# SIMPLE-BuildingSimulation/heat

Measured on AMD Instinct MI355X. Metric: surface-node-updates/sec, higher is better.
Workload: dtype f64

## Files before the change

### heat_amd/csrc/kernels.hip

```cpp
#include <hip/hip_runtime.h>

#include <algorithm>
#include <atomic>
#include <cstdlib>

#include "device_math.hpp"
#include "kernels.hpp"
#include "layout.hpp"

namespace heat {

__device__ __forceinline__ void eval_side(const SideConst &c, const StepWeather &w, double air_t, double rad_alt,
                                          double rad_out, double surf_t, double &hs, double &rad_t, int &bad) {
    const double natural = tarp_natural(air_t, surf_t, c.cos_eff, bad);
    if ((c.kind_n & 3) == KIND_OUTDOOR) {
        const bool windward = (c.kind_n & 4) ? true : ((c.nx * w.sin_wd + c.ny * w.cos_wd) > 0.0);
        const double wf = windward ? 1.0 : 0.5;
        hs = wf * (c.forced * w.sqrt_ws) + natural;
        rad_t = rad_out;
    } else {
        hs = natural;
        rad_t = rad_alt;
    }
}
// ... 18 lines not shown

__device__ __forceinline__ long long side_entry_pos(const SideConst &c) { return __double_as_longlong(c.ambient); }
__device__ __forceinline__ void put_zone_contrib(const SideArrays &sd, const SideConst &c, double hs, double t_face) {
    if ((c.kind_n & 3) == KIND_SPACE) {
        ZoneContrib z;
        z.ha = hs * c.forced;
        z.t_face = t_face;
        sd.zc[side_entry_pos(c)] = z;
    }
}

__device__ __forceinline__ void report_failure(int *flags, int bad, unsigned int index) {
    atomicOr(flags, bad);
    atomicMin(reinterpret_cast<unsigned long long *>(flags + 2), ((unsigned long long)index << 8) | (unsigned int)(bad & 0xff));
}

__device__ __forceinline__ double shfl_f64(double v, int src_lane) { return __shfl(v, src_lane, kWave); }

template <int CTRL>
__device__ __forceinline__ double dpp_rotate_f64(double v) {
    int lo = __double2loint(v), hi = __double2hiint(v);
    lo = __builtin_amdgcn_update_dpp(0, lo, CTRL, 0xf, 0xf, false);
    hi = __builtin_amdgcn_update_dpp(0, hi, CTRL, 0xf, 0xf, false);
    return __hiloint2double(hi, lo);
}
template <int CTRL, int ROW_MASK>
__device__ __forceinline__ double dpp_add_f64(double v) {
    int lo = __double2loint(v), hi = __double2hiint(v);
    lo = __builtin_amdgcn_update_dpp(0, lo, CTRL, ROW_MASK, 0xf, true);
    hi = __builtin_amdgcn_update_dpp(0, hi, CTRL, ROW_MASK, 0xf, true);
    return v + __hiloint2double(hi, lo);
}
__device__ __forceinline__ double wave_sum_f64(double v) {
    v = dpp_add_f64<0x111, 0xf>(v);
    v = dpp_add_f64<0x112, 0xf>(v);
    v = dpp_add_f64<0x114, 0xf>(v);
    v = dpp_add_f64<0x118, 0xf>(v);
    v = dpp_add_f64<0x142, 0xa>(v);
    v = dpp_add_f64<0x143, 0xc>(v);
    const int lo = __builtin_amdgcn_readlane(__double2loint(v), 63);
    const int hi = __builtin_amdgcn_readlane(__double2hiint(v), 63);
    return __hiloint2double(hi, lo);
}

__device__ __forceinline__ double row_sum_f64(double v) {
    v = dpp_add_f64<0x111, 0xf>(v);
    v = dpp_add_f64<0x112, 0xf>(v);
    v = dpp_add_f64<0x114, 0xf>(v);
    v = dpp_add_f64<0x118, 0xf>(v);
    return v;
}

__device__ __forceinline__ double from_prev_lane(double v) { return dpp_rotate_f64<0x13C>(v); }
__device__ __forceinline__ double from_next_lane(double v) { return dpp_rotate_f64<0x134>(v); }

template <int M, bool AFFINE, typename VF, typename QF, typename PUT>
__device__ __forceinline__ void apply_A(const double (&x)[M], VF V, const double (&Ue)[M], double ULe, bool is_first,
                                        bool is_last, double qF, QF qsel, PUT put) {
    const double xl_raw = from_prev_lane(x[M - 1]);
    const double xr_raw = from_next_lane(x[0]);
    const double xl = is_first ? 0.0 : xl_raw;
    const double xr = is_last ? 0.0 : xr_raw;
    double fprev = ULe * (x[0] - xl);
    if (AFFINE) fprev -= qF;
#pragma unroll
    for (int j = 0; j < M; j++) {
        const double xj = x[j];
        double f = Ue[j] * (((j == M - 1) ? xr : x[j + 1]) - xj);
        if (AFFINE) f += qsel(j);
        put(j, V(j) * (f - fprev));
        fprev = f;
    }
}

template <int M, typename VF, typename QF>
__device__ __forceinline__ void rk4_horner(double (&T)[M], VF V, const double (&Ue)[M], double ULe, bool is_first,
                                           bool is_last, double qF, QF qsel) {
    double v[M], z[M];
    apply_A<M, true>(T, V, Ue, ULe, is_first, is_last, qF, qsel, [&](int j, double y) { v[j] = y * (1.0 / 24.0); });
    apply_A<M, false>(v, V, Ue, ULe, is_first, is_last, qF, qsel, [&](int j, double y) { z[j] = 4.0 * v[j] + y; });
    apply_A<M, false>(z, V, Ue, ULe, is_first, is_last, qF, qsel, [&](int j, double y) { z[j] = 12.0 * v[j] + y; });
    apply_A<M, false>(z, V, Ue, ULe, is_first, is_last, qF, qsel,
                      [&](int j, double y) { T[j] = (T[j] + 24.0 * v[j]) + y; });
}

#pragma clang fp contract(off)
constexpr int kSmallNodes = 4;
__device__ __forceinline__ double opaque_select(bool cond, double x, double y) {
    const unsigned long long m = __builtin_amdgcn_ballot_w64(cond);
    int lo, hi;
    asm("v_cndmask_b32 %0, %1, %2, %3" : "=v"(lo) : "v"(__double2loint(y)), "v"(__double2loint(x)), "s"(m));
    asm("v_cndmask_b32 %0, %1, %2, %3" : "=v"(hi) : "v"(__double2hiint(y)), "v"(__double2hiint(x)), "s"(m));
    return __hiloint2double(hi, lo);
}
struct Nodes4 {
    double a, b, c, d;
    __device__ __forceinline__ double get(int j) const { return j == 0 ? +a : (j == 1 ? +b : (j == 2 ? +c : +d)); }
    __device__ __forceinline__ void set(int j, double v) {
        if (j == 0) a = v;
        else if (j == 1) b = v;
        else if (j == 2) c = v;
        else d = v;
    }
    __device__ __forceinline__ double last(int nn) const {
        double r = a;
        r = opaque_select(nn == 2, b, r);
        r = opaque_select(nn == 3, c, r);
        r = opaque_select(nn == 4, d, r);
        return r;
    }
};

template <int CAV>
__device__ __forceinline__ void small_step(const SideConst &cf, const SideConst &cb, const SideDyn &df, const SideDyn &db,
                                           const double *__restrict__ hs_fix, int d, int S, const StepWeather &w,
                                           double t_front_b, double t_back_b, int nn, Nodes4 &T,
                                           const double (&Us)[kSmallNodes], const double (&sol)[kSmallNodes],
                                           const int (&cav)[kSmallNodes], const CavityDev (&cv)[kSmallNodes - 1], int &bad,
                                           unsigned int &iters, SideOut &of, SideOut &ob) {
    constexpr int NS = kSmallNodes;
    const int bk = cb.kind_n & 3;
    auto last = [&](const double (&x)[NS]) {
        double r = x[0];
#pragma unroll
        for (int j = 1; j < NS; j++) r = (j == nn - 1) ? +x[j] : +r;
        return r;
    };
    const double T0 = T.a, Tn = T.last(nn);
    const bool quirk = (bk == KIND_AMBIENT);
    double f_hs, f_rad, b_hs, b_rad;
    const double f_surf = T0, b_surf = quirk ? T0 : Tn;
    eval_side(cf, w, t_front_b, t_front_b, df.rad_t, f_surf, f_hs, f_rad, bad);
    eval_side(cb, w, t_back_b, quirk ? t_front_b : t_back_b, db.rad_t, b_surf, b_hs, b_rad, bad);
    if (f_hs != f_hs || b_hs != b_hs) bad |= FLAG_NAN_HS;
    if (hs_fix != nullptr) {
        const double ff = hs_fix[d], fb = hs_fix[S + d];
        if (ff == ff) f_hs = ff;
        if (fb == fb) b_hs = fb;
    }
    const double f_radhs = rad_hs(cf.emis, f_rad, f_surf);
    const double b_radhs = rad_hs(cb.emis, b_rad, b_surf);

    double old_err = 99999.;
    int count = 0;
    for (;;) {
        double lo[NS], dg[NS], up[NS], q[NS];
#pragma unroll
        for (int j = 0; j < NS; j++) { lo[j] = 0.0; dg[j] = 0.0; up[j] = 0.0; q[j] = 0.0; }
#pragma unroll
        for (int j = 0; j < NS - 1; j++) {
            if (j < nn - 1) {
                double u = Us[j];
                if constexpr (CAV) {
                    if (cav[j] >= 0) u = cavity_u_value(cv[j], T.get(j), T.get(j + 1), bad);
                }
                dg[j] += -u;
                dg[j + 1] = dg[j + 1] - u;
                up[j] = up[j] + u;
                lo[j + 1] = lo[j + 1] + u;
            }
        }
        q[0] += t_front_b * f_hs + f_radhs * (f_rad - T.a);
        dg[0] += -f_hs;
        const double bq = t_back_b * b_hs + b_radhs * (b_rad - T.last(nn));
#pragma unroll
        for (int j = 0; j < NS; j++) {
// ... 128 lines not shown
template <int CAV>
__global__ void __launch_bounds__(256, 2)
k_surfaces_small(const GeneralTile *__restrict__ tiles, int n_tiles, NodeArrays na, int64_t gen_base,
                 SideArrays sd, const CavityDev *__restrict__ cavs,
                 const StepWeather *__restrict__ weather, const int *__restrict__ step_ptr, int step_fixed,
                 const double *__restrict__ zone_T, int *__restrict__ flags,
                 unsigned long long *__restrict__ nomass_iters) {
    const int lane = threadIdx.x & (kWave - 1);
    const int wave = blockIdx.x * (blockDim.x >> 6) + (threadIdx.x >> 6);
    if (wave >= n_tiles) return;
    const GeneralTile tile = tiles[wave];
    const int step = (step_fixed >= 0) ? step_fixed : *step_ptr;
    const StepWeather w = site_weather(weather, sd, tile.surf_base)[step];
    const unsigned int iters = small_tile_march<CAV>(tile.node_base, tile.surf_base, tile.G, lane, na, gen_base, sd, w, zone_T, flags);
    if (lane < tile.G) nomass_iters[(int64_t)wave * kWave + lane] += iters;
}
#pragma clang fp contract(fast)

struct FusedLds {
    double2 *hT;
    double *zT, *za0, *zb0, *zvol;
    double *zsa, *zsb;
    int *zoff;
    unsigned short *slots;
};

constexpr int kFusedBarriersAtInit = 1;
constexpr int kFusedBarriersPerSubstep = 2;

__device__ __forceinline__ void fused_block_init(const FusedBlock &blk, const FusedArgs &fa, const FusedLds &l, int n_threads) {
    const int e_first = fa.zone_eoff[blk.first_zone];
    if ((int)threadIdx.x <= blk.n_zones) l.zoff[threadIdx.x] = fa.zone_eoff[blk.first_zone + threadIdx.x] - e_first;
    if ((int)threadIdx.x < blk.n_zones) {
        const int z = fa.zones[blk.first_zone + threadIdx.x];
        l.zT[threadIdx.x] = fa.zone_T[z];
        l.za0[threadIdx.x] = fa.a0[z];
        l.zb0[threadIdx.x] = fa.b0[z];
        l.zvol[threadIdx.x] = fa.vol[z];
    }
    const int n_e = fa.zone_eoff[blk.first_zone + blk.n_zones] - e_first;
    for (int e = threadIdx.x; e < n_e; e += n_threads) l.slots[fa.slots[e_first + e]] = (unsigned short)e;
    __syncthreads();
}

struct FusedPre {
    int e_first, n_e, zoff, z, slot0;
    double zT, za0, zb0, zvol;
};
__device__ __forceinline__ void fused_pre_a(const FusedBlock &blk, const FusedArgs &fa, FusedPre &p) {
    p = FusedPre{0, 0, 0, 0, 0, 0.0, 0.0, 0.0, 0.0};
    const int nz = blk.n_zones;
    if (nz > 0) {
        p.e_first = fa.zone_eoff[blk.first_zone];
        p.n_e = fa.zone_eoff[blk.first_zone + nz];
        p.zoff = fa.zone_eoff[blk.first_zone + min((int)threadIdx.x, nz)];
        p.z = fa.zones[blk.first_zone + min((int)threadIdx.x, nz - 1)];
    }
}
__device__ __forceinline__ void fused_pre_b(const FusedBlock &blk, const FusedArgs &fa, FusedPre &p) {
    if (blk.n_zones > 0) {
        p.n_e -= p.e_first;
        p.zoff -= p.e_first;
        p.zT = fa.zone_T[p.z];
        p.za0 = fa.a0[p.z];
        p.zb0 = fa.b0[p.z];
        p.zvol = fa.vol[p.z];
        if (p.n_e > 0) p.slot0 = fa.slots[p.e_first + min((int)threadIdx.x, p.n_e - 1)];
    }
}
__device__ __forceinline__ void fused_block_init(const FusedBlock &blk, const FusedArgs &fa, const FusedLds &l, int n_threads,
                                                 const FusedPre &p) {
    if ((int)threadIdx.x <= blk.n_zones) l.zoff[threadIdx.x] = p.zoff;
    if ((int)threadIdx.x < blk.n_zones) {
        l.zT[threadIdx.x] = p.zT;
        l.za0[threadIdx.x] = p.za0;
        l.zb0[threadIdx.x] = p.zb0;
        l.zvol[threadIdx.x] = p.zvol;
    }
    if ((int)threadIdx.x < p.n_e) l.slots[p.slot0] = (unsigned short)threadIdx.x;
    for (int e = threadIdx.x + n_threads; e < p.n_e; e += n_threads) l.slots[fa.slots[p.e_first + e]] = (unsigned short)e;
    __syncthreads();
}

struct TeamCtx {
    int team, member, round, it;
    int *flags;
};
__device__ __forceinline__ unsigned long long team_granule(unsigned int data, unsigned int tag) {
    return ((unsigned long long)tag << 32) | data;
}
template <int TEAM>
__device__ __forceinline__ void fused_zone_phase(const FusedBlock &blk, const FusedArgs &fa, const FusedLds &l, int wib,
                                                 int n_waves, int lane, int &bad_all, const TeamCtx &tc_) {
    __syncthreads();
    auto team_area = [&](int j, unsigned int &mask, unsigned int &tag) -> unsigned long long * {
        const unsigned int info = fa.team_zinfo[blk.first_zone + j];
        mask = info >> 16;
        tag = fa.tag_base | ((unsigned int)tc_.round << 12) | (unsigned int)(tc_.it + 1);
        return fa.xbuf + ((((size_t)tc_.team * 2 + (tc_.it & 1)) * kTeamZones + (info & 0xffffu)) * kTeamMax) * 4;
    };
    auto publish = [&](int j, double a, double b) {
        unsigned int mask, tag;
        unsigned long long *g = team_area(j, mask, tag) + tc_.member * 4;
        const unsigned long long ab = (unsigned long long)__double_as_longlong(a), bb = (unsigned long long)__double_as_longlong(b);
        __hip_atomic_store(g + 0, team_granule((unsigned int)ab, tag), __ATOMIC_RELAXED, __HIP_MEMORY_SCOPE_AGENT);
        __hip_atomic_store(g + 1, team_granule((unsigned int)(ab >> 32), tag), __ATOMIC_RELAXED, __HIP_MEMORY_SCOPE_AGENT);
        __hip_atomic_store(g + 2, team_granule((unsigned int)bb, tag), __ATOMIC_RELAXED, __HIP_MEMORY_SCOPE_AGENT);
        __hip_atomic_store(g + 3, team_granule((unsigned int)(bb >> 32), tag), __ATOMIC_RELAXED, __HIP_MEMORY_SCOPE_AGENT);
    };
    auto gather = [&](int j, double &a, double &b) {
        unsigned int mask, tag;
        const unsigned long long *area = team_area(j, mask, tag);
        double sa = 0.0, sb = 0.0;
        for (int m = 0; m < kTeamMax; m++) {
            if (!((mask >> m) & 1u)) continue;
            double am = a, bm = b;
            if (m != tc_.member) {
                const unsigned long long *g = area + m * 4;
                unsigned long long g0 = 0, g1 = 0, g2 = 0, g3 = 0;
                bool got = false;
                for (int spin = 0; spin < (1 << 21); spin++) {
                    g0 = __hip_atomic_load(g + 0, __ATOMIC_RELAXED, __HIP_MEMORY_SCOPE_AGENT);
                    g1 = __hip_atomic_load(g + 1, __ATOMIC_RELAXED, __HIP_MEMORY_SCOPE_AGENT);
                    g2 = __hip_atomic_load(g + 2, __ATOMIC_RELAXED, __HIP_MEMORY_SCOPE_AGENT);
                    g3 = __hip_atomic_load(g + 3, __ATOMIC_RELAXED, __HIP_MEMORY_SCOPE_AGENT);
                    got = (unsigned int)(g0 >> 32) == tag && (unsigned int)(g1 >> 32) == tag &&
                          (unsigned int)(g2 >> 32) == tag && (unsigned int)(g3 >> 32) == tag;
                    if (got) break;
                    __builtin_amdgcn_s_sleep(4);
                }
                if (!got) atomicOr(tc_.flags, FLAG_EXCHANGE);
                am = __longlong_as_double((long long)((g0 & 0xffffffffull) | (g1 << 32)));
                bm = __longlong_as_double((long long)((g2 & 0xffffffffull) | (g3 << 32)));
            }
            sa += am;
            sb += bm;
        }
        a = sa;
        b = sb;
    };
    auto finish = [&](int j, double a, double b, double tc, double cz) {
        a += l.za0[j];
        b += l.zb0[j];
        double ft = tc;
        if (fabs(b) > 1e-9) ft = a / b + (tc - a / b) * exp(-b * fa.dt / cz);
        if (ft != ft) bad_all |= FLAG_NAN_ZONE;
        l.zT[j] = ft;
    };
    if (blk.n_zones <= n_waves) {
        if (wib < blk.n_zones) {
            const int j = wib;
            const int e0 = l.zoff[j], e1 = l.zoff[j + 1];
            const double tc = l.zT[j];
            const double cz = zone_mcp(l.zvol[j], tc);
            double a = 0.0, b = 0.0;
            for (int e = e0 + lane; e < e1; e += kWave) {
                const double2 ht = l.hT[e];
                a += ht.x * ht.y;
                b += ht.x;
            }
            a = wave_sum_f64(a);
            b = wave_sum_f64(b);
            if (lane == 0) {
                if constexpr (TEAM) {
                    publish(j, a, b);
                    gather(j, a, b);
                }
                finish(j, a, b, tc, cz);
            }
        }
    } else {
        const int row = lane >> 4, rl = lane & 15;
        const bool one_pass = blk.n_zones <= 4 * n_waves;
        (void)one_pass;
#pragma clang loop unroll(disable)
        for (int j0 = 0; j0 < blk.n_zones; j0 += 4 * n_waves) {
            const int j = j0 + 4 * wib + row;
            const bool on = j < blk.n_zones;
            const int jj = on ? j : 0;
            const int e0 = l.zoff[jj], e1 = on ? l.zoff[jj + 1] : e0;
            const double tc = l.zT[jj];
            const double cz = zone_mcp(l.zvol[jj], tc);
            double a = 0.0, b = 0.0;
            for (int e = e0 + rl; __any(e < e1); e += 16) {
                if (e < e1) {
                    const double2 ht = l.hT[e];
                    a += ht.x * ht.y;
                    b += ht.x;
                }
            }
            a = row_sum_f64(a);
            b = row_sum_f64(b);
            if constexpr (TEAM) {
                if (on && rl == 15) {
                    publish(j, a, b);
                    if (one_pass) {
                        gather(j, a, b);
                        finish(j, a, b, tc, cz);
                    } else {
                        l.zsa[j] = a;
                        l.zsb[j] = b;
                    }
                }
            } else {
                if (on && rl == 15) finish(j, a, b, tc, cz);
            }
        }
        if constexpr (TEAM) {
            if (!one_pass) {
#pragma clang loop unroll(disable)
                for (int j0 = 0; j0 < blk.n_zones; j0 += 4 * n_waves) {
                    const int j = j0 + 4 * wib + row;
                    if (j < blk.n_zones && rl == 15) {
                        const double tc = l.zT[j];
                        const double cz = zone_mcp(l.zvol[j], tc);
                        double a = l.zsa[j], b = l.zsb[j];
                        gather(j, a, b);
                        finish(j, a, b, tc, cz);
                    }
                }
            }
        }
    }
    __syncthreads();
}

#pragma clang fp contract(off)
__device__ void fused_small_wave(const FusedBlock &blk, const FusedArgs &fa, const FusedLds &l, int lanes_per_side,
                                 int wib, int n_waves, int lane, const NodeArrays &na, const SideArrays &sd,
                                 const StepWeather *__restrict__ weather, int *__restrict__ flags) {
    const int tile_index = blk.first_small + (wib - blk.n_tiles);
    const GeneralTile tile = fa.gen_tiles[tile_index];
// ... 11 lines not shown
    Nodes4 T{0.0, 0.0, 0.0, 0.0};
    double Us[kSmallNodes], sol[kSmallNodes];
    int cav[kSmallNodes];
    CavityDev cv[kSmallNodes - 1];
    small_load<1>(tile, active ? lane : 0, na, fa.gen_base, df, db, nn, T, Us, sol, cav, cv);
    fused_block_init(blk, fa, l, n_waves * kWave);
    int bad_all = 0;
    unsigned int iters = 0;
    SideOut of{0.0, 0.0}, ob{0.0, 0.0};
    auto btemp = [&](const SideConst &c, int lz, const StepWeather &w) -> double {
        const int kind = c.kind_n & 3;
        if (kind == KIND_SPACE) return l.zT[lz];
        if (kind == KIND_AMBIENT) return c.ambient;
        return w.t_out;
    };
#pragma clang loop unroll(disable)
    for (int it = 0; it < fa.n_sub; it++) {
        const StepWeather w = weather[it];
        int bad = 0;
        small_step<1>(cf, cb, df, db, sd.hs_fix, d, S, w, btemp(cf, lz_f, w), btemp(cb, lz_b, w), nn, T, Us, sol, cav,
                      cv, bad, iters, of, ob);
        if (active) {
            bad_all |= bad;
            const double Tl = T.last(nn);
            if ((cf.kind_n & 3) == KIND_SPACE) l.hT[l.slots[wib * kWave + lane]] = make_double2(of.hs * area, T.a);
            if ((cb.kind_n & 3) == KIND_SPACE) l.hT[l.slots[lanes_per_side + wib * kWave + lane]] = make_double2(ob.hs * area, Tl);
        }
        fused_zone_phase<0>(blk, fa, l, wib, n_waves, lane, bad_all, TeamCtx{0, 0, 0, 0, nullptr});
    }
    if ((int)threadIdx.x < blk.n_zones) fa.zone_T[fa.zones[blk.first_zone + threadIdx.x]] = l.zT[threadIdx.x];
    if (active) {
        double *Tg = na.T + tile.node_base + lane;
#pragma unroll
        for (int j = 0; j < kSmallNodes; j++) if (j < nn) Tg[(int64_t)j * kWave] = T.get(j);
        sd.out[d] = of;
        sd.out[S + d] = ob;
        if (fa.small_iters) fa.small_iters[(int64_t)tile_index * kWave + lane] += iters;
    }
    if (bad_all) report_failure(flags, bad_all, (unsigned int)d);
}
#pragma clang fp contract(fast)

#ifdef HEAT_STAMPS
constexpr int kStampsPerBlock = 8;
__device__ unsigned long long g_stamps[65536 * kStampsPerBlock];
#define HEAT_STAMP(k, real)                                                                                   \
    do {                                                                                                      \
        if constexpr (FUSED) {                                                                                \
            if (threadIdx.x == 0 && (counter_index >> 2) < 65536)                                             \
                g_stamps[(counter_index >> 2) * kStampsPerBlock + (k)] =                                      \
                    (real) ? __builtin_amdgcn_s_memrealtime() : __builtin_amdgcn_s_memtime();                 \
        }                                                                                                     \
    } while (0)
#else
#define HEAT_STAMP(k, real) do { } while (0)
#endif
#ifdef HEAT_STREAM_STAMPS
#ifndef HEAT_STAMPS
constexpr int kStampsPerBlock = 8;
__device__ unsigned long long g_stamps[65536 * kStampsPerBlock];
#endif
#define HEAT_SSTAMP(k, drain)                                                                                  \
    do {                                                                                                       \
        if constexpr (!FUSED && PAL) {                                                                         \
            if (drain) asm volatile("s_waitcnt vmcnt(0) lgkmcnt(0)" ::: "memory");                             \
            if (lane == 0 && counter_index < 32768)                                                            \
                g_stamps[(counter_index + (M == 16 ? 32768 : 0)) * kStampsPerBlock + (k)] = __builtin_amdgcn_s_memtime(); \
        }                                                                                                      \
    } while (0)
#else
#define HEAT_SSTAMP(k, drain) do { } while (0)
#endif

template <int M, int NM, int PAL, int CAV, int FUSED, int SMALL = 0>
__device__ __forceinline__ void fast_tile_march(const FastTile tile, int counter_index, bool nm_on, int lane, int wib,
                                                double *s_pal, double *s_V, double *s_pos, const FusedLds &fl, const FusedBlock &blk,
                                                int blk_waves, int n_it, int step0, const NodeArrays &na,
                                                const SideArrays &sd, const StepWeather *__restrict__ weather,
                                                const double *__restrict__ zone_T, int *__restrict__ flags,
                                                unsigned long long *__restrict__ nomass_iters, const FusedArgs &fa,
                                                bool write_out = true, const TeamCtx team = TeamCtx{0, 0, 0, 0, nullptr}) {
    constexpr int kLanes = (FUSED ? FUSED : 4) * kWave;
    constexpr bool kVinLds = FUSED && M == 16;
    HEAT_STAMP(4, true);
    HEAT_STAMP(0, false);
    HEAT_SSTAMP(0, false);
    double2 *const s_hT = fl.hT;
    double *const s_zT = fl.zT;
    (void)s_hT; (void)s_zT; (void)s_V; (void)s_pos; (void)nm_on; (void)blk; (void)blk_waves; (void)counter_index;
    FusedPre pre;
    (void)pre;
    if constexpr (FUSED) fused_pre_a(blk, fa, pre);
    const bool mixed = PAL && (tile.k & kTileMixedBit) != 0;
    constexpr bool kChunks = NM == 2 && PAL;
    const bool chunky = kChunks && (tile.k & kTileChunkyBit) != 0;
    const int k = tile.k & 0xff;
    const bool full = (tile.k & 0x100) != 0;
    const int G = tile.G;
    const int Lk = mixed ? k : (kWave / k) * k;
    int g = (int)(((float)lane + 0.5f) * (1.0f / (float)k));
    int seg = lane - g * k;
    bool is_last = (seg == k - 1);
    const bool in_layout = lane < Lk;
    if (mixed) {
        const unsigned int e = reinterpret_cast<const unsigned short *>(na.cls + tile.node_base + (int64_t)M * Lk)[in_layout ? lane : 0];
        g = (int)(e & 63u);
        seg = (int)((e >> 6) & 63u);
        is_last = (e & (unsigned int)kLaneLastBit) != 0;
    }
    const bool active = in_layout && (g < G);
    if (!active) g = 0;
    const int d = tile.surf_base + g;
    const int ll = in_layout ? lane : 0;

    const int S = sd.S;
    const bool is_first = (seg == 0);
    constexpr bool kSingleLane = !FUSED || (M == 8 && !CAV);
    const bool single = kSingleLane && is_first && is_last;
    const bool my_back = !is_first;
    const int sidx = (my_back ? S : 0) + d;
    const SideConst c_load = sd.sc[sidx];
    const SideDyn dy_load = sd.dyn[sidx];
    SideConst cb2 = c_load;
    SideDyn db2 = dy_load;
    if constexpr (kSingleLane) {
        if ((!mixed && k == 1) || single) {
            cb2 = sd.sc[S + d];
            db2 = sd.dyn[S + d];
        }
    }
    int4 cavref = make_int4(-1, -1, -1, -1);
    if constexpr (CAV) cavref = reinterpret_cast<const int4 *>(na.cavref)[d];
    const int kind_n_mine = c_load.kind_n;
    if constexpr (!FUSED) s_pos[threadIdx.x] = c_load.ambient;
    int my_lz = 0, b_lz = 0;
    double my_area = 0.0;
    if constexpr (FUSED) {
        my_lz = fa.side_lzone[sidx];
        my_area = fa.side_area[sidx];
        if constexpr (kSingleLane) b_lz = single ? fa.side_lzone[S + d] : 0;
    }
    (void)b_lz;
    int peer_lz = 0;
    if constexpr (FUSED) peer_lz = fa.side_lzone[d];
    (void)peer_lz;

    double T[M], V[M], U[M];
    unsigned int cw[M / 4];
    (void)cw;
    if constexpr (PAL) {
        const int pstride = na.pal_stride;
        const int ubase = na.pal_ubase;
        double *sp = s_pal + wib * (kWave * pstride);
        auto load_cls_T = [&]() {
            const unsigned char *pc = na.cls + tile.node_base + (int64_t)ll * M;
            if constexpr (M == 4) {
                cw[0] = *reinterpret_cast<const unsigned int *>(pc);
            } else {
#pragma unroll
                for (int q = 0; q < M / 8; q++) {
                    const uint2 w0 = reinterpret_cast<const uint2 *>(pc)[q];
                    cw[2 * q] = w0.x;
                    cw[2 * q + 1] = w0.y;
                }
            }
            const double2 *pT = reinterpret_cast<const double2 *>(na.T + tile.node_base);
#pragma unroll
            for (int jp = 0; jp < M / 2; jp++) {
                const double2 t = pT[jp * Lk + ll];
                T[2 * jp] = t.x; T[2 * jp + 1] = t.y;
            }
        };
        if constexpr (FUSED) {
            load_cls_T();
            fused_pre_b(blk, fa, pre);
        }
        {
            const double2 *gp = reinterpret_cast<const double2 *>(na.pal + (int64_t)tile.surf_base * pstride);
            double2 *sp2 = reinterpret_cast<double2 *>(sp);
            const int n2 = G * (pstride / 2);
            for (int i0 = 0; i0 < n2; i0 += 6 * kWave) {
                double2 t6[6];
#pragma unroll
                for (int q = 0; q < 6; q++) t6[q] = gp[min(i0 + q * kWave + lane, n2 - 1)];
                if constexpr (FUSED) {
                    asm volatile("" : "+v"(t6[0].x), "+v"(t6[1].x), "+v"(t6[2].x), "+v"(t6[3].x), "+v"(t6[4].x), "+v"(t6[5].x),
                                      "+v"(pre.zT), "+v"(pre.za0), "+v"(pre.zb0), "+v"(pre.zvol), "+v"(pre.slot0));
                }
#pragma unroll
                for (int q = 0; q < 6; q++)
                    if (i0 + q * kWave + lane < n2) sp2[i0 + q * kWave + lane] = t6[q];
            }
        }
        if constexpr (!FUSED) load_cls_T();
        HEAT_STAMP(6, false);
        __builtin_amdgcn_wave_barrier();
        {
            const double *mp = sp + g * pstride;
#pragma unroll
            for (int j = 0; j < M; j++) {
                const unsigned int cbj = (cw[j >> 2] >> (8 * (j & 3))) & 0xff;
                const unsigned int vi = cbj & (kPalV - 1);
                V[j] = mp[vi >= kPalVMark1 ? 0u : vi];
                U[j] = mp[ubase + ((cbj >> kPalUShift) & (kPalU - 1))];
            }
        }
        if constexpr (kVinLds) {
#pragma unroll
            for (int j = 0; j < M; j++) s_V[j * kLanes + threadIdx.x] = V[j];
        }
    } else {
        const double2 *pT = reinterpret_cast<const double2 *>(na.T + tile.node_base);
        const double2 *pV = reinterpret_cast<const double2 *>(na.V + tile.node_base);
        const double2 *pU = reinterpret_cast<const double2 *>(na.U + tile.node_base);
#pragma unroll
        for (int jp = 0; jp < M / 2; jp++) {
            const double2 t = pT[jp * Lk + ll];
            const double2 v = pV[jp * Lk + ll];
            const double2 u = pU[jp * Lk + ll];
            T[2 * jp] = t.x; T[2 * jp + 1] = t.y;
            V[2 * jp] = v.x; V[2 * jp + 1] = v.y;
            U[2 * jp] = u.x; U[2 * jp + 1] = u.y;
        }
    }
    HEAT_STAMP(7, false);
    if constexpr (FUSED) fused_block_init(blk, fa, fl, blk_waves * kWave, pre);

    const int first_lane = lane - seg;
    const int nn = kind_n_mine >> 16;
    const int jl = full ? (M - 1) : (nn - 1 - (mixed ? seg : k - 1) * M);

    auto pick_last = [&](const double (&x)[M]) {
        double r = x[M - 1];
        if (!full) {
#pragma unroll
            for (int j = 0; j < M - 1; j++) r = (j == jl) ? +x[j] : +r;
        }
        return r;
    };

    const bool wave_quirk = __any((is_last && (kind_n_mine & 3) == KIND_AMBIENT && my_back) ||
                                  (single && ((kind_n_mine >> 4) & 3) == KIND_AMBIENT));
    double zt_mine = 0.0, zt_b2 = 0.0;
    (void)zt_mine; (void)zt_b2;
    if constexpr (!FUSED) {
        zt_mine = zone_T[c_load.zone];
        if constexpr (kSingleLane) zt_b2 = zone_T[cb2.zone];
    }

    auto Vat = [&](int j) -> double {
        if constexpr (kVinLds) return s_V[j * kLanes + threadIdx.x];
        else return V[j];
    };
    auto V_last = [&]() {
        double r = Vat(M - 1);
        if (!full) {
#pragma unroll
            for (int j = 0; j < M - 1; j++) r = (j == jl) ? Vat(j) : r;
        }
        return r;
    };

    int bad_all = 0;
    unsigned int nm_passes = 0;
    double o_hs = 0.0, o_flow = 0.0, o2_hs = 0.0, o2_flow = 0.0;
    StepWeather w_next = weather[step0];

    HEAT_STAMP(1, false);
    HEAT_SSTAMP(1, true);
    SideConst c_cur = c_load;
    SideDyn dy_cur = dy_load;
#pragma clang loop unroll(disable)
    for (int it = 0; it < n_it; it++) {
    const StepWeather w = w_next;
    if constexpr (FUSED) w_next = weather[min(it + 1, n_it - 1)];
    const SideConst c = c_cur;
    const SideDyn dy = dy_cur;
    auto btemp = [&](const SideConst &cc, int lz, double zt) -> double {
        const int kind = cc.kind_n & 3;
        if (kind == KIND_SPACE) {
            if constexpr (FUSED) return s_zT[lz];
            else return zt;
        }
        if (kind == KIND_AMBIENT) return cc.ambient;
        return w.t_out;
    };

    int bad = 0;
    auto prepare = [&](const SideConst &cc, const SideDyn &dd, bool back, int rec, int lz, double zt, double &air_t,
                       double &rad_t, double &forced, bool &use_front_T) {
        const int kind = cc.kind_n & 3;
        air_t = btemp(cc, lz, zt);
        rad_t = air_t;
        use_front_T = false;
        forced = 0.0;
        if (kind == KIND_OUTDOOR) {
            const bool windward = (cc.kind_n & 4) ? true : ((cc.nx * w.sin_wd + cc.ny * w.cos_wd) > 0.0);
            forced = (windward ? 1.0 : 0.5) * (cc.forced * w.sqrt_ws);
            rad_t = dd.rad_t;
        } else if (back && kind == KIND_AMBIENT) {
            const int fkind = (cc.kind_n >> 4) & 3;
            if (fkind == KIND_SPACE) {
                if constexpr (FUSED) rad_t = s_zT[peer_lz];
                else rad_t = zt;
            } else if (fkind == KIND_AMBIENT) {
                rad_t = cc.forced;
            } else {
                rad_t = w.t_out;
            }
            use_front_T = true;
        }
        (void)rec;
    };
    auto conv = [&](double air_t, double forced, double nat_pos, double nat_neg, int rec, double surf_t) {
        double hs = forced + tarp_natural_coef(air_t, surf_t, nat_pos, nat_neg, bad);
        if (hs != hs) bad |= FLAG_NAN_HS;
        if (sd.hs_fix != nullptr) {
            const double fix = sd.hs_fix[rec];
            if (fix == fix) hs = fix;
        }
        return hs;
    };
// ... 120 lines not shown
                for (int j = 0; j < M; j++) {
                    ta = (j == j0) ? +T[j] : +ta;
                    tb = (j == j1) ? +T[j] : +tb;
                    if (j + 1 < M) tp = (j + 1 == j0) ? +T[j] : +tp;
                    if (j > 0) tn = (j == j1 + 1) ? +T[j] : +tn;
                    if (j + 1 < M) up = (j + 1 == j0) ? +U[j] : +up;
                    ui = (j == j0) ? +U[j] : +ui;
                    un = (j == j1) ? +U[j] : +un;
                }
                const bool faceL = is_first && j0 == 0;
                const bool faceR = is_last && j1 == jl;
                const double hL = faceL ? fF_hs : up, hR = faceR ? fB_hs : un;
                const double solA = faceL ? fF_sol : 0.0;
                const double solB = faceR ? fB_sol : 0.0;
                double old_err = 99999.;
                int count = 0;
                for (;;) {
                    const double t_last = (cn == 2) ? tb : ta;
                    const double qL = faceL ? (fF_air * fF_hs + fF_rhs * (fF_rad - ta)) : (up * tp);
                    const double qR = faceR ? (fB_air * fB_hs + fB_rhs * (fB_rad - t_last)) : (un * tn);
                    double x0, x1 = 0.0, err;
                    if (cn == 1) {
                        const double dg = (0.0 + -hL) + -hR;
                        const double q = (((0.0 + qL) + qR) + (solA + solB)) * -1.;
                        x0 = q / dg;
                        err = fabs(x0 - ta);
                    } else {
                        const double u = ui;
                        double dg0 = 0.0 + -u, dg1 = 0.0 - u;
                        const double up0 = 0.0 + u, lo1 = 0.0 + u;
                        dg0 += -hL;
                        dg1 += -hR;
                        const double q0 = ((0.0 + qL) + solA) * -1.;
                        double q1 = ((0.0 + qR) + solB) * -1.;
                        const double f = lo1 / dg0;
                        dg1 -= f * up0;
                        q1 -= f * q0;
                        x1 = q1 / dg1;
                        x0 = (q0 - up0 * x1) / dg0;
                        err = fabs(x0 - ta) + fabs(x1 - tb);
                    }
                    nm_passes++;
                    if (err > old_err) break;
                    if (err != err) { bad |= FLAG_NAN_NOMASS; break; }
                    ta = (ta + x0) * 0.5;
                    if (cn == 2) tb = (tb + x1) * 0.5;
                    const double tol = (count < 100) ? 0.01 : 0.5;
                    if (err / (double)cn < tol) break;
                    old_err = err;
                    count++;
                }
#pragma unroll
                for (int j = 0; j < M; j++) {
                    T[j] = (j == j0) ? ta : T[j];
                    if (j > 0) T[j] = (cn == 2 && j == j1) ? tb : T[j];
                }
            }
        }
    }

    if constexpr (CAV) {
        const double T_next_first = from_next_lane(T[0]);
#pragma unroll
        for (int r = 0; r < 2; r++) {
            const int node = r ? cavref.z : cavref.x;
            const int cidx = r ? cavref.w : cavref.y;
            const int jc = node - seg * M;
            if (active && cidx >= 0 && jc >= 0 && jc < M) {
                double ta = T[0], tb = T_next_first;
#pragma unroll
                for (int j = 0; j < M; j++) {
                    ta = (j == jc) ? +T[j] : +ta;
                    if (j + 1 < M) tb = (j == jc) ? +T[j + 1] : +tb;
                }
                const double u = cavity_u_value(na.cavs[cidx], ta, tb, bad);
#pragma unroll
                for (int j = 0; j < M; j++) U[j] = (j == jc) ? u : U[j];
            }
        }
        UL = from_prev_lane(U[M - 1]);
        if (is_first) UL = 0.0;
    }

    {
        const double hBe = is_last ? hB : 0.0;
        if (full) {
            U[M - 1] = is_last ? hB : U[M - 1];
        } else {
#pragma unroll
            for (int j = 0; j < M; j++) U[j] = (j == jl) ? U[j] + hBe : U[j];
        }
        const double ULe = is_first ? hF : UL;
        const double qFe = is_first ? qF : 0.0;
        const double qBe = is_last ? qB : 0.0;
#ifdef HEAT_STREAM_STAMPS
        asm volatile("" : "+v"(T[0]), "+v"(T[M - 1]));
        HEAT_SSTAMP(6, false);
#endif
        if (full) {
            rk4_horner<M>(T, Vat, U, ULe, is_first, is_last, qFe, [&](int j) -> double { return (j == M - 1) ? qBe : 0.0; });
        } else {
            rk4_horner<M>(T, Vat, U, ULe, is_first, is_last, qFe, [&](int j) -> double { return (j == jl) ? qBe : 0.0; });
        }
#ifdef HEAT_STREAM_STAMPS
        asm volatile("" : "+v"(T[0]), "+v"(T[M - 1]));
        HEAT_SSTAMP(7, false);
#endif
        if constexpr (FUSED) {
            if (full) {
                U[M - 1] = is_last ? 0.0 : U[M - 1];
            } else {
#pragma unroll
                for (int j = 0; j < M; j++) U[j] = (is_last && j == jl) ? 0.0 : U[j];
            }
        }
    }

    if constexpr (!FUSED) {
        if (active) {
            double2 *pT = reinterpret_cast<double2 *>(na.T + tile.node_base);
#pragma unroll
            for (int jp = 0; jp < M / 2; jp++) pT[jp * Lk + lane] = make_double2(T[2 * jp], T[2 * jp + 1]);
        }
    }

    const double T0n = wave_quirk ? shfl_f64(T[0], first_lane) : T[0];
    const double Tln = pick_last(T);
    const double Tnn = Tln;
    {
        const double surf_t = (my_back && !my_useF) ? Tnn : T0n;
        const double hs = conv(my_air, my_forced, c.cos_eff, c.alpha, sidx, surf_t);
        const double face_t = my_back ? Tln : T[0];
        o_hs = hs;
        o_flow = (face_t - my_air) * hs;
        if constexpr (!FUSED) {
            if (active && (is_first || is_last) && (kind_n_mine & 3) == KIND_SPACE) {
                ZoneContrib z;
                z.ha = hs * c.forced;
                z.t_face = face_t;
                sd.zc[__double_as_longlong(s_pos[threadIdx.x])] = z;
            }
        }
        if constexpr (FUSED) {
            if (active && (is_first || is_last) && (c.kind_n & 3) == KIND_SPACE)
                s_hT[fl.slots[(my_back ? kLanes : 0) + wib * kWave + lane]] = make_double2(hs * my_area, face_t);
        }
    }
    if (single) {
        const double hs = conv(b_air, b_forced, b_cos, b_neg, S + d, b_useF ? T0n : Tnn);
        o2_hs = hs;
        o2_flow = (Tln - b_air) * hs;
        if constexpr (!FUSED) {
            if (active) put_zone_contrib(sd, cb2, hs, Tln);
        } else {
            if (active && (cb2.kind_n & 3) == KIND_SPACE)
                s_hT[fl.slots[kLanes + wib * kWave + lane]] = make_double2(hs * my_area, Tln);
        }
    } else if (!(is_first || is_last)) {
        bad = 0;
    }
    bad_all |= bad;

    if constexpr (FUSED) {
        int sidx_next = sidx;
        asm volatile("" : "+v"(sidx_next));
        c_cur = sd.sc[sidx_next];
        dy_cur = sd.dyn[sidx_next];
        if constexpr (SMALL == 2) {
            TeamCtx tcx = team;
            tcx.it = it;
            fused_zone_phase<1>(blk, fa, fl, wib, blk_waves, lane, bad_all, tcx);
        } else {
            fused_zone_phase<0>(blk, fa, fl, wib, blk_waves, lane, bad_all, team);
        }
    }
    }
    HEAT_STAMP(2, false);
    HEAT_SSTAMP(2, false);

    if constexpr (FUSED) {
        if (active) {
            double2 *pT = reinterpret_cast<double2 *>(na.T + tile.node_base);
#pragma unroll
            for (int jp = 0; jp < M / 2; jp++) pT[jp * Lk + lane] = make_double2(T[2 * jp], T[2 * jp + 1]);
        }
        if (threadIdx.x < blk.n_zones) fa.zone_T[fa.zones[blk.first_zone + threadIdx.x]] = s_zT[threadIdx.x];
    }
    if (write_out && active && (is_first || is_last)) {
        SideOut o;
        o.hs = o_hs;
        o.flow = o_flow;
        sd.out[sidx] = o;
    }
    if (write_out && single && active) {
        SideOut o;
        o.hs = o2_hs;
        o.flow = o2_flow;
        sd.out[S + d] = o;
    }
    if (active && bad_all) report_failure(flags, bad_all, (unsigned int)d);
#ifdef HEAT_STAMPS
    asm volatile("s_waitcnt vmcnt(0)" ::: "memory");
#endif
    HEAT_STAMP(3, false);
    HEAT_SSTAMP(3, true);
    HEAT_STAMP(5, true);
    if constexpr (NM) {
        unsigned int tot = nm_passes;
#pragma unroll
        for (int o = kWave / 2; o > 0; o >>= 1) tot += __shfl_down(tot, o, kWave);
        if (lane == 0 && tot) nomass_iters[counter_index] += tot;
    }
}

template <int M, int NM, int PAL, int CAV, int FUSED, int SMALL = 0>
__global__ void __launch_bounds__(FUSED ? 64 * FUSED : 256, (FUSED || (M == 16 && !CAV)) ? 2 : 1)
k_surfaces_fast(const FastTile *__restrict__ tiles, int n_tiles, NodeArrays na, SideArrays sd,
                const StepWeather *__restrict__ weather, const int *__restrict__ step_ptr, int step_fixed,
                const double *__restrict__ zone_T, int *__restrict__ flags,
                unsigned long long *__restrict__ nomass_iters, FusedArgs fa) {
    static_assert(!FUSED || (PAL && !(CAV && M == 16)),
                  "the cluster-resident march exists for palette classes; with gas cavities for 4 or 8 nodes per lane");
    constexpr int kMaxW = FUSED ? FUSED : 4;
    constexpr int kLanes = kMaxW * kWave;
    extern __shared__ double s_dyn[];
    __shared__ double s_pos_static[FUSED ? 2 : kLanes];
    double *const s_pal = s_dyn;
    constexpr bool kVinLds = FUSED && M == 16;
    double *const s_V = s_dyn + kLanes * na.pal_stride;
    FusedLds fl;
    fl.hT = reinterpret_cast<double2 *>(s_V + (kVinLds ? M : 0) * kLanes);
    fl.zT = reinterpret_cast<double *>(fl.hT) + 4 * kLanes;
    fl.za0 = fl.zT + kFusedMaxZones;
    fl.zb0 = fl.za0 + kFusedMaxZones;
    fl.zvol = fl.zb0 + kFusedMaxZones;
    fl.zsa = fl.zvol + kFusedMaxZones;
    fl.zsb = fl.zsa + kFusedMaxZones;
    fl.zoff = reinterpret_cast<int *>(fl.zsb + kFusedMaxZones);
    fl.slots = reinterpret_cast<unsigned short *>(fl.zoff + kFusedMaxZones + 2);
    const int lane = threadIdx.x & (kWave - 1);
    const int wib = threadIdx.x >> 6;
    int wave0 = blockIdx.x * (blockDim.x >> 6) + wib;
    int n_waves = gridDim.x * (blockDim.x >> 6);
    FusedBlock blk{0, 0, 0, 0, 0, 0};
    int blk_waves = 0;
    int bi = blockIdx.x;
    __shared__ int s_next_block;
    const int n_it = FUSED ? fa.n_sub : 1;
    const int step0 = FUSED ? 0 : ((step_fixed >= 0) ? step_fixed : *step_ptr);
    const bool write_out = FUSED || step_fixed >= 0 || step0 == step_ptr[1];
    constexpr bool kTeam = FUSED && SMALL == 2;
    TeamCtx team{0, 0, 0, 0, flags};
    int sb = 0, n_teams = 1;
    if constexpr (kTeam) {
        team.team = (int)blockIdx.x / fa.team_size;
        team.member = (int)blockIdx.x % fa.team_size;
        n_teams = (int)gridDim.x / fa.team_size;
        sb = team.team;
    }
    for (int wave = wave0; FUSED ? (kTeam ? (sb < fa.n_super) : (bi < fa.n_blocks)) : (wave < n_tiles); wave += n_waves) {
    if constexpr (FUSED) {
        if constexpr (kTeam) {
            const FusedSuper su = fa.supers[fa.reverse ? fa.n_super - 1 - sb : sb];
            if (team.member >= su.n_members) {
                sb += n_teams;
                team.round++;
                continue;
            }
            bi = su.first_block + team.member;
        }
        blk = fa.blocks[(!kTeam && fa.reverse) ? fa.n_blocks - 1 - bi : bi];
        blk_waves = blk.n_tiles + (SMALL == 1 ? blk.n_small : 0);
        const bool looping = kTeam || fa.queue != nullptr;
        if (wib >= blk_waves) {
            if (!looping) return;
            for (int q = 0; q < kFusedBarriersAtInit; q++) __syncthreads();
            for (int it = 0; it < fa.n_sub; it++)
                for (int q = 0; q < kFusedBarriersPerSubstep; q++) __syncthreads();
            goto next_block;
        }
        if constexpr (SMALL == 1) {
            if (wib >= blk.n_tiles) {
                fused_small_wave(blk, fa, fl, kLanes, wib, blk_waves, lane, na, sd, weather, flags);
                if (!looping) return;
                goto next_block;
            }
        }
        wave = blk.first_tile + wib;
    }
    {
    const int tix = (!FUSED && fa.reverse) ? n_tiles - 1 - wave : wave;
    const FastTile tl = tiles[tix];
    fast_tile_march<M, NM, PAL, CAV, FUSED, SMALL>(tl, tix, true, lane, wib, s_pal, s_V, s_pos_static, fl, blk, blk_waves, n_it, step0, na,
                                                   sd, site_weather(weather, sd, tl.surf_base), zone_T, flags, nomass_iters, fa,
                                                   write_out, team);
    }
next_block:
    if constexpr (FUSED) {
        if constexpr (kTeam) {
            __syncthreads();
            sb += n_teams;
            team.round++;
        } else {
            if (fa.queue == nullptr) break;
            __syncthreads();
            if (threadIdx.x == 0) s_next_block = (int)(gridDim.x + atomicAdd(fa.queue, 1u));
            __syncthreads();
            bi = s_next_block;
        }
    }
    }
}

constexpr int kTileKindShift = 9;
// ... 514 lines not shown
__global__ void __launch_bounds__(256)
k_outputs_compact(int n_surf, int n_zones, const SideOut *__restrict__ out, const int32_t *__restrict__ orig_of,
                  const double *__restrict__ zone_T, double *__restrict__ dst) {
    const int i = blockIdx.x * blockDim.x + threadIdx.x;
    if (i < n_surf) {
        const SideOut f = out[i], b = out[n_surf + i];
        double2 *p = reinterpret_cast<double2 *>(dst + 4 * (int64_t)orig_of[i]);
        p[0] = make_double2(f.hs, b.hs);
        p[1] = make_double2(f.flow, b.flow);
    }
    if (i < n_zones) dst[4 * (int64_t)n_surf + i] = zone_T[i];
}

__global__ void k_set_step(int *step_ptr, int v, int last) {
    step_ptr[0] = v;
    step_ptr[1] = last;
}

__global__ void k_begin_march(const StepWeather *__restrict__ h_weather, StepWeather *__restrict__ weather, int n_records,
                              const double *__restrict__ h_zone_ab, double *__restrict__ a0, double *__restrict__ b0,
                              int n_zones, int *step_ptr, int last) {
    const int i = blockIdx.x * blockDim.x + threadIdx.x;
    if (i < n_records) weather[i] = h_weather[i];
    if (i < n_zones) {
        a0[i] = h_zone_ab[i];
        b0[i] = h_zone_ab[n_zones + i];
    }
    if (i == 0) {
        step_ptr[0] = 0;
        step_ptr[1] = last;
    }
}

static inline int blocks_for_waves(int n_waves) { return (n_waves + 3) / 4; }
static inline size_t pal_lds_bytes(const NodeArrays &na) { return (size_t)4 * kWave * na.pal_stride * sizeof(double); }

void launch_surfaces_fast(int M, int nm, int pal, int cav, double grid_share, const FastTile *tiles, int n_tiles,
                          const NodeArrays &na,
                          const SideArrays &sa, const StepWeather *weather, const int *step_ptr, int step_fixed,
                          const double *zone_T, int *flags, unsigned long long *nomass_iters, int n_cu, hipStream_t st, int reverse) {
    if (n_tiles <= 0) return;
    static const int tune = getenv("HEAT_AMD_PERSIST") ? atoi(getenv("HEAT_AMD_PERSIST")) : 1;
    const int blocks_per_cu = (M == 4 ? 5 : (M == 8 ? 3 : 2)) * tune;
    const int full_grid = blocks_for_waves(n_tiles);
    const bool persistent = tune > 0 && grid_share > 0.999 && M >= 8;
    const dim3 grid(persistent ? std::min(full_grid, n_cu * blocks_per_cu) : full_grid), block(256);
    FusedArgs no_fa{};
    no_fa.reverse = reverse;
#define HEAT_LAUNCH_FAST(MM, NN, PP, CC)                                                                          \
    hipLaunchKernelGGL((k_surfaces_fast<MM, NN, PP, CC, 0>), grid, block, PP ? pal_lds_bytes(na) : 0, st, tiles, n_tiles, na, sa, weather, \
                       step_ptr, step_fixed, zone_T, flags, nomass_iters, no_fa)
#define HEAT_LAUNCH_M(MM)                                     \
    switch ((nm ? 3 : 0) + (cav ? 2 : (pal ? 1 : 0))) {       \
    case 0: HEAT_LAUNCH_FAST(MM, 0, 0, 0); break;             \
    case 1: HEAT_LAUNCH_FAST(MM, 0, 1, 0); break;             \
    case 2: HEAT_LAUNCH_FAST(MM, 0, 1, 1); break;             \
    case 3: HEAT_LAUNCH_FAST(MM, 1, 0, 0); break;             \
    case 4: if (nm == 2) HEAT_LAUNCH_FAST(MM, 2, 1, 0); else HEAT_LAUNCH_FAST(MM, 1, 1, 0); break; \
    default: if (nm == 2) HEAT_LAUNCH_FAST(MM, 2, 1, 1); else HEAT_LAUNCH_FAST(MM, 1, 1, 1); break; \
    }
    if (M == 4) { HEAT_LAUNCH_M(4) } else if (M == 8) { HEAT_LAUNCH_M(8) } else { HEAT_LAUNCH_M(16) }
#undef HEAT_LAUNCH_M
#undef HEAT_LAUNCH_FAST
}

void launch_surfaces_stream(int variant, const FastTile *tiles, int n_tiles, const NodeArrays &na, int64_t gen_base, const SideArrays &sa,
                            const StepWeather *weather, const int *step_ptr, int step_fixed, const double *zone_T,
                            int *flags, unsigned long long *nomass_iters, int n_cu, hipStream_t st, int reverse) {
    if (n_tiles <= 0) return;
    static const int per_cu_env = getenv("HEAT_AMD_STREAM_BLOCKS") ? atoi(getenv("HEAT_AMD_STREAM_BLOCKS")) : 0;
    const int per_cu = per_cu_env > 0 ? per_cu_env : (variant == kStreamLight ? 3 : 2);
    const int grid = std::min(blocks_for_waves(n_tiles), n_cu * per_cu);
#define HEAT_LAUNCH_STREAM(V)                                                                                       \
    hipLaunchKernelGGL(k_surfaces_stream<V>, dim3(grid), dim3(256), pal_lds_bytes(na), st, tiles, n_tiles, na, gen_base, sa, weather, \
                       step_ptr, step_fixed, zone_T, flags, nomass_iters, reverse)
    if (variant == kStreamWide) HEAT_LAUNCH_STREAM(kStreamWide);
    else if (variant == kStreamLight) HEAT_LAUNCH_STREAM(kStreamLight);
    else if (variant == kStreamChunks) HEAT_LAUNCH_STREAM(kStreamChunks);
    else HEAT_LAUNCH_STREAM(kStreamCav);
#undef HEAT_LAUNCH_STREAM
}

size_t fused_lds_bytes(int max_waves, int M, int pal_stride) {
    return (size_t)max_waves * kWave * ((pal_stride + (M == 16 ? M : 0)) * sizeof(double) + 2 * sizeof(double2)) +
           6 * kFusedMaxZones * sizeof(double) + (kFusedMaxZones + 2) * sizeof(int) + kFusedMaxEntries * sizeof(uint16_t);
}

template <int MM, int NN, int CC, int FW, int SM>
static hipError_t launch_fused_one(int grid_blocks, const FastTile *tiles, int n_tiles, const NodeArrays &na,
                                   const SideArrays &sa, const StepWeather *weather, int *flags,
                                   unsigned long long *nomass_iters, const FusedArgs &fa, hipStream_t st) {
    const size_t lds = fused_lds_bytes(FW, MM, na.pal_stride);
    constexpr int kMaxDevices = 64;
    static std::atomic<size_t> attr_bytes[kMaxDevices];
    if (lds > 160 * 1024) return hipErrorInvalidValue;
    int dev = 0;
    if (hipGetDevice(&dev) != hipSuccess || dev < 0 || dev >= kMaxDevices) dev = kMaxDevices - 1;
    if (lds > 64 * 1024 && lds > attr_bytes[dev].load(std::memory_order_acquire)) {
        hipError_t e = hipFuncSetAttribute(reinterpret_cast<const void *>(&k_surfaces_fast<MM, NN, 1, CC, FW, SM>),
                                           hipFuncAttributeMaxDynamicSharedMemorySize, (int)lds);
        if (e != hipSuccess) return e;
        if (dev != kMaxDevices - 1) attr_bytes[dev].store(lds, std::memory_order_release);
    }
    hipLaunchKernelGGL((k_surfaces_fast<MM, NN, 1, CC, FW, SM>), dim3(grid_blocks), dim3(kWave * FW), lds, st, tiles,
                       n_tiles, na, sa, weather, nullptr, 0, nullptr, flags, nomass_iters, fa);
    return hipSuccess;
}

int fused_blocks_per_cu(int M, int cav, int mixed, int max_waves, int pal_stride) {
    const int waves_per_simd = (M == 4 && !cav && !mixed) ? 3 : 2;
    const int by_regs = std::max(1, waves_per_simd * 4 / max_waves);
    const int by_lds = std::max<int>(1, (int)(160 * 1024 / fused_lds_bytes(max_waves, M, pal_stride)));
    return std::min(by_regs, by_lds);
}

template <int MM, int NN>
static int team_occupancy(size_t lds) {
    int n = 0;
    if (hipOccupancyMaxActiveBlocksPerMultiprocessor(&n, reinterpret_cast<const void *>(&k_surfaces_fast<MM, NN, 1, 0, 4, 2>),
                                                     kWave * 4, lds) != hipSuccess)
        return 0;
    return n;
}
int fused_team_blocks_per_cu(int M, int nm, int pal_stride) {
    const size_t lds = fused_lds_bytes(4, M, pal_stride);
    if (M == 4) return nm ? team_occupancy<4, 1>(lds) : team_occupancy<4, 0>(lds);
    if (M == 8) return nm ? team_occupancy<8, 1>(lds) : team_occupancy<8, 0>(lds);
    return nm ? team_occupancy<16, 1>(lds) : team_occupancy<16, 0>(lds);
}

hipError_t launch_surfaces_fused(int M, int nm, int cav, int mixed, int max_waves, int grid_blocks, const FastTile *tiles,
                                 int n_tiles, const NodeArrays &na, const SideArrays &sa, const StepWeather *weather,
                                 int *flags, unsigned long long *nomass_iters, const FusedArgs &fa, hipStream_t st) {
    const int n_blocks = grid_blocks;
    if (n_blocks <= 0) return hipSuccess;
    if (cav && M == 16) return hipErrorInvalidValue;
#define HEAT_FUSED(MM, NN, CC, FW, SM) \
    launch_fused_one<MM, NN, CC, FW, SM>(n_blocks, tiles, n_tiles, na, sa, weather, flags, nomass_iters, fa, st)
    if (mixed == 2) {
        if (cav || max_waves > 4) return hipErrorInvalidValue;
        if (M == 4) return nm ? HEAT_FUSED(4, 1, 0, 4, 2) : HEAT_FUSED(4, 0, 0, 4, 2);
        if (M == 8) return nm ? HEAT_FUSED(8, 1, 0, 4, 2) : HEAT_FUSED(8, 0, 0, 4, 2);
        return nm ? HEAT_FUSED(16, 1, 0, 4, 2) : HEAT_FUSED(16, 0, 0, 4, 2);
    }
    if (mixed) {
        if (M == 4) return max_waves <= 4 ? HEAT_FUSED(4, 1, 1, 4, 1) : HEAT_FUSED(4, 1, 1, 8, 1);
        if (M == 8) return max_waves <= 4 ? HEAT_FUSED(8, 1, 1, 4, 1) : HEAT_FUSED(8, 1, 1, 8, 1);
        return max_waves <= 4 ? HEAT_FUSED(16, 1, 0, 4, 1) : HEAT_FUSED(16, 1, 0, 8, 1);
    }
    if (nm == 2 && !cav && M <= 8) {
        if (M == 4) return max_waves <= 4 ? HEAT_FUSED(4, 2, 0, 4, 0) : HEAT_FUSED(4, 2, 0, 8, 0);
        return max_waves <= 4 ? HEAT_FUSED(8, 2, 0, 4, 0) : HEAT_FUSED(8, 2, 0, 8, 0);
    }
#define HEAT_FUSED_NW(MM, CC)                                                    \
    (max_waves <= 4 ? (nm ? HEAT_FUSED(MM, 1, CC, 4, 0) : HEAT_FUSED(MM, 0, CC, 4, 0)) \
                    : (nm ? HEAT_FUSED(MM, 1, CC, 8, 0) : HEAT_FUSED(MM, 0, CC, 8, 0)))
    if (M == 4) return cav ? HEAT_FUSED_NW(4, 1) : HEAT_FUSED_NW(4, 0);
    if (M == 8) return cav ? HEAT_FUSED_NW(8, 1) : HEAT_FUSED_NW(8, 0);
    return HEAT_FUSED_NW(16, 0);
#undef HEAT_FUSED_NW
#undef HEAT_FUSED
}

void launch_surfaces_general(const GeneralTile *tiles, int n_tiles, const NodeArrays &na, int64_t gen_base,
                             const SideArrays &sa, const CavityDev *cavs, double *scratch,
                             const StepWeather *weather, const int *step_ptr, int step_fixed,
                             const double *zone_T, int *flags, unsigned long long *nomass_iters, hipStream_t st) {
// ... 117 lines not shown
```

Measured before the change: 499.8 billion.

## Use difference-form RK4 operator and per-wave zone reduction for single-zone fused blocks

Rewrites the RK4 Horner operator in the fused path into a difference form with precomputed coefficients (a_j = V_j*U_{j-1}, c_j = V_j*U_j). This removes per-node flux subtraction and the multiply by V in each of the four apply passes. It also adds a single-zone fast path: each wave reduces its zone heat contributions in registers and writes one partial sum to LDS, so the per-slot hT scatter and the later per-zone gather are skipped. The cost is an extra LDS row per lane for the last V value and a different floating-point evaluation order.

```diff
diff --git a/heat_amd/csrc/kernels.hip b/heat_amd/csrc/kernels.hip
--- a/heat_amd/csrc/kernels.hip
+++ b/heat_amd/csrc/kernels.hip
@@ -124,6 +124,37 @@
     apply_A<M, false>(z, V, Ue, ULe, is_first, is_last, qF, qsel, [&](int j, double y) { z[j] = 12.0 * v[j] + y; });
     apply_A<M, false>(z, V, Ue, ULe, is_first, is_last, qF, qsel,
                       [&](int j, double y) { T[j] = (T[j] + 24.0 * v[j]) + y; });
+}
+
+template <int M, bool AFFINE, typename AF, typename SF, typename PUT>
+__device__ __forceinline__ void apply_A_diff(const double (&x)[M], AF a, const double (&c)[M], double a0, bool is_first,
+                                             bool is_last, double sF, SF ssel, PUT put) {
+    const double xl_raw = from_prev_lane(x[M - 1]);
+    const double xr_raw = from_next_lane(x[0]);
+    const double xl = is_first ? 0.0 : xl_raw;
+    const double xr = is_last ? 0.0 : xr_raw;
+    double dprev = x[0] - xl;
+#pragma unroll
+    for (int j = 0; j < M; j++) {
+        const double dj = ((j == M - 1) ? xr : x[j + 1]) - x[j];
+        double y;
+        if (AFFINE) y = c[j] * dj + ((j == 0) ? sF + ssel(0) : ssel(j));
+        else y = c[j] * dj;
+        y -= ((j == 0) ? a0 : a(j)) * dprev;
+        put(j, y);
+        dprev = dj;
+    }
+}
+
+template <int M, typename AF, typename SF>
+__device__ __forceinline__ void rk4_horner_diff(double (&T)[M], AF a, const double (&c)[M], double a0, bool is_first,
+                                                bool is_last, double sF, SF ssel) {
+    double v[M], z[M];
+    apply_A_diff<M, true>(T, a, c, a0, is_first, is_last, sF, ssel, [&](int j, double y) { v[j] = y * (1.0 / 24.0); });
+    apply_A_diff<M, false>(v, a, c, a0, is_first, is_last, sF, ssel, [&](int j, double y) { z[j] = 4.0 * v[j] + y; });
+    apply_A_diff<M, false>(z, a, c, a0, is_first, is_last, sF, ssel, [&](int j, double y) { z[j] = 12.0 * v[j] + y; });
+    apply_A_diff<M, false>(z, a, c, a0, is_first, is_last, sF, ssel,
+                           [&](int j, double y) { T[j] = (T[j] + 24.0 * v[j]) + y; });
 }
 
 #pragma clang fp contract(off)
@@ -418,6 +449,12 @@
     __syncthreads();
 }
 
+__device__ __forceinline__ bool fused_one_zone(const FusedBlock &blk, int n_waves) {
+#ifdef HEAT_XP_NO_ONE_ZONE
+    return false;
+#endif
+    return blk.n_zones == 1 && n_waves == blk.n_tiles;
+}
 struct TeamCtx {
     int team, member, round, it;
     int *flags;
@@ -428,6 +465,12 @@
 template <int TEAM>
 __device__ __forceinline__ void fused_zone_phase(const FusedBlock &blk, const FusedArgs &fa, const FusedLds &l, int wib,
                                                  int n_waves, int lane, int &bad_all, const TeamCtx &tc_) {
+    const bool one_zone = !TEAM && fused_one_zone(blk, n_waves);
+    double tc1 = 0.0, cz1 = 0.0;
+    if (one_zone && wib == 0) {
+        tc1 = l.zT[0];
+        cz1 = zone_mcp(l.zvol[0], tc1);
+    }
     __syncthreads();
     auto team_area = [&](int j, unsigned int &mask, unsigned int &tag) -> unsigned long long * {
         const unsigned int info = fa.team_zinfo[blk.first_zone + j];
@@ -483,7 +526,16 @@
         if (ft != ft) bad_all |= FLAG_NAN_ZONE;
         l.zT[j] = ft;
     };
-    if (blk.n_zones <= n_waves) {
+    if (one_zone) {
+        if (wib == 0 && lane == 0) {
+            double a = l.zsa[0], b = l.zsb[0];
+            for (int w = 1; w < n_waves; w++) {
+                a += l.zsa[w];
+                b += l.zsb[w];
+            }
+            finish(0, a, b, tc1, cz1);
+        }
+    } else if (blk.n_zones <= n_waves) {
         if (wib < blk.n_zones) {
             const int j = wib;
             const int e0 = l.zoff[j], e1 = l.zoff[j + 1];
@@ -661,6 +713,13 @@
                                                 bool write_out = true, const TeamCtx team = TeamCtx{0, 0, 0, 0, nullptr}) {
     constexpr int kLanes = (FUSED ? FUSED : 4) * kWave;
     constexpr bool kVinLds = FUSED && M == 16;
+#ifdef HEAT_XP_NO_DIFF
+    constexpr bool kDiff = false;
+#else
+    constexpr bool kDiff = FUSED && !NM && !CAV;
+#endif
+    double *const s_Vl = kDiff ? s_V + (kVinLds ? M : 0) * kLanes : nullptr;
+    (void)s_Vl;
     HEAT_STAMP(4, true);
     HEAT_STAMP(0, false);
     HEAT_SSTAMP(0, false);
@@ -784,7 +843,7 @@
                 U[j] = mp[ubase + ((cbj >> kPalUShift) & (kPalU - 1))];
             }
         }
-        if constexpr (kVinLds) {
+        if constexpr (kVinLds && !kDiff) {
 #pragma unroll
             for (int j = 0; j < M; j++) s_V[j * kLanes + threadIdx.x] = V[j];
         }
@@ -817,6 +876,19 @@
         }
         return r;
     };
+
+    if constexpr (kDiff) {
+        s_Vl[threadIdx.x] = pick_last(V);
+        const double Up_raw = from_prev_lane(U[M - 1]);
+        const double Up = is_first ? 1.0 : Up_raw;
+#pragma unroll
+        for (int j = M - 1; j >= 0; j--) {
+            const double aj = V[j] * ((j == 0) ? Up : U[j - 1]);
+            U[j] = V[j] * U[j];
+            if constexpr (kVinLds) s_V[j * kLanes + threadIdx.x] = aj;
+            else V[j] = aj;
+        }
+    }
 
     const bool wave_quirk = __any((is_last && (kind_n_mine & 3) == KIND_AMBIENT && my_back) ||
                                   (single && ((kind_n_mine >> 4) & 3) == KIND_AMBIENT));
@@ -1103,7 +1175,35 @@
         if (is_first) UL = 0.0;
     }
 
-    {
+    if constexpr (kDiff) {
+        const double a0s = kVinLds ? s_V[threadIdx.x] : V[0];
+        const double Vl = s_Vl[threadIdx.x];
+        const double a0e = is_first ? a0s * hF : a0s;
+        const double sF = is_first ? a0s * qF : 0.0;
+        const double sB = is_last ? Vl * qB : 0.0;
+        const double cBe = is_last ? Vl * hB : 0.0;
+        if (full) {
+            U[M - 1] = is_last ? cBe : U[M - 1];
+        } else {
+#pragma unroll
+            for (int j = 0; j < M; j++) U[j] = (j == jl) ? U[j] + cBe : U[j];
+        }
+        auto Aat = [&](int j) -> double {
+            if constexpr (kVinLds) return s_V[j * kLanes + threadIdx.x];
+            else return V[j];
+        };
+        if (full) {
+            rk4_horner_diff<M>(T, Aat, U, a0e, is_first, is_last, sF, [&](int j) -> double { return (j == M - 1) ? sB : 0.0; });
+        } else {
+            rk4_horner_diff<M>(T, Aat, U, a0e, is_first, is_last, sF, [&](int j) -> double { return (j == jl) ? sB : 0.0; });
+        }
+        if (full) {
+            U[M - 1] = is_last ? 0.0 : U[M - 1];
+        } else {
+#pragma unroll
+            for (int j = 0; j < M; j++) U[j] = (is_last && j == jl) ? 0.0 : U[j];
+        }
+    } else {
         const double hBe = is_last ? hB : 0.0;
         if (full) {
             U[M - 1] = is_last ? hB : U[M - 1];
@@ -1148,6 +1248,9 @@
     const double T0n = wave_quirk ? shfl_f64(T[0], first_lane) : T[0];
     const double Tln = pick_last(T);
     const double Tnn = Tln;
+    const bool one_zone = FUSED && SMALL != 2 && fused_one_zone(blk, blk_waves);
+    double za = 0.0, zb = 0.0;
+    (void)one_zone;
     {
         const double surf_t = (my_back && !my_useF) ? Tnn : T0n;
         const double hs = conv(my_air, my_forced, c.cos_eff, c.alpha, sidx, surf_t);
@@ -1163,8 +1266,15 @@
             }
         }
         if constexpr (FUSED) {
-            if (active && (is_first || is_last) && (c.kind_n & 3) == KIND_SPACE)
-                s_hT[fl.slots[(my_back ? kLanes : 0) + wib * kWave + lane]] = make_double2(hs * my_area, face_t);
+            if (active && (is_first || is_last) && (c.kind_n & 3) == KIND_SPACE) {
+                const double hsa = hs * my_area;
+                if (one_zone) {
+                    za = hsa * face_t;
+                    zb = hsa;
+                } else {
+                    s_hT[fl.slots[(my_back ? kLanes : 0) + wib * kWave + lane]] = make_double2(hsa, face_t);
+                }
+            }
         }
     }
     if (single) {
@@ -1174,8 +1284,15 @@
         if constexpr (!FUSED) {
             if (active) put_zone_contrib(sd, cb2, hs, Tln);
         } else {
-            if (active && (cb2.kind_n & 3) == KIND_SPACE)
-                s_hT[fl.slots[kLanes + wib * kWave + lane]] = make_double2(hs * my_area, Tln);
+            if (active && (cb2.kind_n & 3) == KIND_SPACE) {
+                const double hsa = hs * my_area;
+                if (one_zone) {
+                    za += hsa * Tln;
+                    zb += hsa;
+                } else {
+                    s_hT[fl.slots[kLanes + wib * kWave + lane]] = make_double2(hsa, Tln);
+                }
+            }
         }
     } else if (!(is_first || is_last)) {
         bad = 0;
@@ -1187,6 +1304,14 @@
         asm volatile("" : "+v"(sidx_next));
         c_cur = sd.sc[sidx_next];
         dy_cur = sd.dyn[sidx_next];
+        if (one_zone) {
+            za = wave_sum_f64(za);
+            zb = wave_sum_f64(zb);
+            if (lane == kWave - 1) {
+                fl.zsa[wib] = za;
+                fl.zsb[wib] = zb;
+            }
+        }
         if constexpr (SMALL == 2) {
             TeamCtx tcx = team;
             tcx.it = it;
@@ -1250,7 +1375,7 @@
     constexpr bool kVinLds = FUSED && M == 16;
     double *const s_V = s_dyn + kLanes * na.pal_stride;
     FusedLds fl;
-    fl.hT = reinterpret_cast<double2 *>(s_V + (kVinLds ? M : 0) * kLanes);
+    fl.hT = reinterpret_cast<double2 *>(s_V + ((kVinLds ? M : 0) + (FUSED ? 1 : 0)) * kLanes);
     fl.zT = reinterpret_cast<double *>(fl.hT) + 4 * kLanes;
     fl.za0 = fl.zT + kFusedMaxZones;
     fl.zb0 = fl.za0 + kFusedMaxZones;
@@ -1931,7 +2056,7 @@
 }
 
 size_t fused_lds_bytes(int max_waves, int M, int pal_stride) {
-    return (size_t)max_waves * kWave * ((pal_stride + (M == 16 ? M : 0)) * sizeof(double) + 2 * sizeof(double2)) +
+    return (size_t)max_waves * kWave * ((pal_stride + (M == 16 ? M : 0) + 1) * sizeof(double) + 2 * sizeof(double2)) +
            6 * kFusedMaxZones * sizeof(double) + (kFusedMaxZones + 2) * sizeof(int) + kFusedMaxEntries * sizeof(uint16_t);
 }
 
```

Result: slower. 493.0 billion (median of 2 runs) (-1.4%).
